# shyam196/egc

Hardware: AMD Instinct MI355X
Metric: EGC-M layer fwd edges/sec on ogbn-arxiv; achieved HBM GB/s vs roofline (higher is better)
Workload: dtype f32

## Files before the change

egc_amd/csrc/egc_aggregate.hip:

```cpp
#include <stdlib.h>

#include <algorithm>

#include "egc_aggregate_dev.h"
#include "egc_pack_map.h"

namespace egc {

bool stdvar_reference(const egc_layer* layer) {
  const char* e = getenv("EGC_STDVAR_REFERENCE");
  if (layer == nullptr || e == nullptr || e[0] == '\0' || (e[0] == '0' && e[1] == '\0')) return false;
  for (int t = 0; t < layer->num_aggrs && t < EGC_MAX_AGGRS; ++t)
    if (layer->aggrs[t] == EGC_AGGR_VAR || layer->aggrs[t] == EGC_AGGR_STD) return true;
  return false;
}

template <int CHUNKS>
__device__ inline void set_shift(const AggArgs& a, __amdgpu_buffer_rsrc_t rsrc, int row, int lane, Acc<CHUNKS>& acc) {
  bool need = false;
  for (int t = 0; t < a.A; ++t) need = need || a.aggr[t] == EGC_AGGR_VAR || a.aggr[t] == EGC_AGGR_STD;
  if (!need && a.stats == nullptr) return;
  if (a.var_ref) return;
  const int rs = __builtin_amdgcn_readfirstlane(a.rowptr[row]), re = __builtin_amdgcn_readfirstlane(a.rowptr[row + 1]);
  if (re <= rs) return;
  const int first = __builtin_amdgcn_readfirstlane(a.col[rs]);
  const int q = lane & ((1 << a.lpr_log2) - 1);
#pragma unroll
  for (int k = 0; k < CHUNKS; ++k) {
    const int s = k * 64 + q;
    acc.sh[k] = load_slot(rsrc, s < a.slots ? (unsigned)first * (unsigned)a.ldb * 4u + (unsigned)s * 16u : OOB);
  }
}

template <int CHUNKS, int U>
__device__ inline void accumulate_range(const AggArgs& a, __amdgpu_buffer_rsrc_t rsrc, int row, int start, int end,
                                        int lane, Acc<CHUNKS>& acc, int& nself) {
  const int G = 64 >> a.lpr_log2;
// ... 661 lines not shown
  PlanCaps caps = plan_caps(n, e);
  a.rows_per_wave = 0;
  a.n_chunks_hint = (graph->n_chunks >= 0 && graph->n_chunks <= caps.cap_chunks) ? (int)graph->n_chunks : -1;
  const bool force_generic = getenv("EGC_FORCE_GENERIC") != nullptr || a.var_ref != 0;
  if (!force_generic && fast_path_supported(a, layer->weight_layout, chunks)) {
    if (arg_done != nullptr) *arg_done = true;
    return launch_fast(a, n, caps, stream);
  }

  switch (chunks) {
    case 1: return launch_all<1>(a, n, caps, wpb, lds_bytes, stream);
    case 2: return launch_all<2>(a, n, caps, wpb, lds_bytes, stream,
                                 !force_generic && getenv("EGC_NO_WIDE") == nullptr && wide_path_supported(a, layer->weight_layout));
    case 3: return launch_all<3>(a, n, caps, wpb, lds_bytes, stream);
    case 4: return launch_all<4>(a, n, caps, wpb, lds_bytes, stream);
    default: return EGC_ERR_UNSUPPORTED;
  }
}

int egc_layer_forward_f32(const egc_graph* graph, const egc_layer* layer, const float* x, const float* wcat,
                          const float* bcat, const float* bias, float* bases, int32_t ldb, float* weightings,
                          float* out, void* workspace, size_t workspace_bytes, egc_stream_t stream) {
  if (graph == nullptr) return EGC_ERR_INVALID;
  int st = validate_layer(layer);
  if (st != EGC_OK) return st;
  const int fg = layer->num_bases * layer_basis_stride(layer);
  const int w = layer->num_heads * layer->num_bases * layer->num_aggrs;
  st = egc_basis_transform_f32(x, wcat, bcat, graph->n_nodes, layer->in_channels, fg, w, bases, ldb, weightings, stream);
  if (st != EGC_OK) return st;
  return egc_aggregate_combine_f32(graph, layer, bases, ldb, weightings, bias, out, nullptr, nullptr, workspace,
                                   workspace_bytes, stream);
}

int egc_layer_forward_packed(const egc_graph* graph, const egc_layer* layer, const float* x, const void* packed,
                             const float* bcat, const float* bias, float* bases, int32_t ldb, float* weightings,
                             float* out, void* workspace, size_t workspace_bytes, egc_stream_t stream) {
  if (graph == nullptr) return EGC_ERR_INVALID;
  int st = validate_layer(layer);
  if (st != EGC_OK) return st;
  const int fg = layer->num_bases * layer_basis_stride(layer);
  const int w = layer->num_heads * layer->num_bases * layer->num_aggrs;
  st = egc_basis_transform_packed_ex(x, packed, bcat, graph->n_nodes, layer->in_channels, fg, w, egc_layer_gemm_flags(layer),
                                     bases, ldb, weightings, stream);
  if (st != EGC_OK) return st;
  return egc_aggregate_combine_f32(graph, layer, bases, ldb, weightings, bias, out, nullptr, nullptr, workspace,
                                   workspace_bytes, stream);
}

static int tile_layer_args(const egc_layer* layer, AggArgs& a, bool two_sets_ok = false) {
  int st = validate_layer(layer);
  if (st != EGC_OK) return st;
  a = AggArgs{};
  a.ldb = egc_bases_ld(layer);
  a.slots = a.ldb / 4;
  a.F_out = layer->out_channels;
  a.H = layer->num_heads;
  a.B = layer->num_bases;
  a.A = layer->num_aggrs;
  a.L = layer->out_channels / layer->num_heads;
  a.Ls = layer_basis_stride(layer);
  a.W = a.H * a.B * a.A;
  a.ldw = a.W;
  for (int t = 0; t < EGC_MAX_AGGRS; ++t) a.aggr[t] = t < a.A ? layer->aggrs[t] : 0;
  a.x_looped = layer->agg_set == EGC_SET_LOOPED;
  a.y_looped = layer->sym_set == EGC_SET_LOOPED;
  a.loops_all = layer->loops_all_nodes != 0;
  if (layer->weight_layout == EGC_LAYOUT_HAB) { a.sa = a.B; a.sb = 1; } else { a.sa = 1; a.sb = a.A; }
  a.act = layer->weight_act;
  a.lpr_log2 = 4;
  int chunks = a.slots <= 64 ? 1 : (a.slots + 63) / 64;
  a.n_nodes = 1;
  if (!fast_path_supported(a, layer->weight_layout, chunks) && !(two_sets_ok && wide_path_supported(a, layer->weight_layout)))
    return EGC_ERR_UNSUPPORTED;
  return EGC_OK;
// ... 230 lines not shown
```

egc_amd/csrc/egc_aggregate_fast.hip:

```cpp
#include <stdlib.h>

#include "egc_aggregate_fast_dev.h"

namespace egc {

template <int LPR_LOG2, int HPB, int NEED, class C>
#ifndef EGC_AGG_WAVES_SQ
#define EGC_AGG_WAVES_SQ 5
#endif
__global__ void __launch_bounds__(256) __attribute__((amdgpu_waves_per_eu(NEED == 0 ? EGC_AGG_WAVES : ((NEED & NEED_ARG) && (NEED & NEED_SQ)) ? 2 : (NEED == NEED_SQ || NEED == NEED_MN) ? EGC_AGG_WAVES_SQ : 4)))
agg_fast_kernel(AggArgs a) {
  constexpr int LPR = 1 << LPR_LOG2, G = 64 / LPR;
  extern __shared__ float smem[];
  if ((int)blockIdx.x < a.chunk_blocks && (int)blockIdx.x * 4 >= a.plan[1]) return;
  const int wave = __builtin_amdgcn_readfirstlane(threadIdx.x >> 6);
  const int lane = threadIdx.x & 63;
  const int g = lane >> LPR_LOG2;
  const int q = lane & (LPR - 1);
  const unsigned slot_off = (unsigned)q * 16u;
  const unsigned row_bytes = (unsigned)a.ldb * 4u;
  const bool lane_live = q < C::slots(a);
  const int F_out = C::F_out(a);
  float* lds_bias = smem + wave * a.lds_floats_per_wave;
  const bool post = a.post_scale != nullptr;
// ... 483 lines not shown
  const int lpr = a.slots <= 16 ? 16 : a.slots <= 32 ? 32 : 64;
  const int G = 64 / lpr;
  a.lanes_pb = a.Ls / 4;
  a.magic_P = (unsigned)(((uint64_t)1 << 32) / (uint64_t)a.lanes_pb) + 1u;
  if ((a.lanes_pb & (a.lanes_pb - 1)) == 0) {
    int lg = 0;
    while ((4 << lg) < a.Ls) ++lg;
    a.lpb_log2 = lg;
  } else {
    a.lpb_log2 = -1;
  }
  if (a.rows_per_wave <= 0) a.rows_per_wave = (G == 1 && (int64_t)a.row_end - a.row_begin >= 32768) ? 4 : 1;
  if (a.rows_per_wave * G > 60) a.rows_per_wave = 60 / G;
  a.chunk_blocks = (int)ceil_div(a.n_chunks_hint >= 0 ? a.n_chunks_hint : caps.cap_chunks, 4);
  a.need_mean = a.need_var = 0;
  int need = 0;
  for (int t = 0; t < a.A; ++t) {
    if (a.aggr[t] == EGC_AGGR_MEAN || a.aggr[t] == EGC_AGGR_VAR || a.aggr[t] == EGC_AGGR_STD) a.need_mean = 1;
    if (a.aggr[t] == EGC_AGGR_VAR || a.aggr[t] == EGC_AGGR_STD) { a.need_var = 1; need |= NEED_SQ; }
    if (a.aggr[t] == EGC_AGGR_MIN) need |= NEED_MN;
  }
  a.w_lds_stride = (a.W + 3) & ~3;
  a.bias_lds_floats = (a.H * a.Ls + 3) & ~3;
  a.lds_floats_per_wave = (a.post_scale != nullptr ? 2 : 1) * a.bias_lds_floats + G * a.w_lds_stride;
  size_t lds = (size_t)4 * a.lds_floats_per_wave * sizeof(float);
  if (lds > 64 * 1024) return EGC_ERR_UNSUPPORTED;
  const int64_t row_blocks = ceil_div((int64_t)a.row_end - a.row_begin, (int64_t)4 * a.rows_per_wave * G);
  const unsigned grid = (unsigned)(a.chunk_blocks + row_blocks);

  if (getenv("EGC_NO_STATIC_CFG") == nullptr) {
    int status = EGC_OK;
    constexpr int S = EGC_AGGR_SUM, M = EGC_AGGR_MEAN, X = EGC_AGGR_MAX, Y = EGC_AGGR_SYMNORM;
    EGC_STATIC_CFG(8, 4, 16, 4, agg_pack(S, M, X, Y), EGC_ACT_NONE, true, true, true, 0)
    EGC_STATIC_CFG(8, 4, 16, 4, agg_pack(S, EGC_AGGR_STD, X, Y), EGC_ACT_NONE, true, true, true, NEED_SQ)
    EGC_STATIC_CFG(8, 4, 16, 1, agg_pack(Y), EGC_ACT_NONE, true, true, true, 0)
    EGC_STATIC_CFG(8, 4, 16, 3, agg_pack(Y, X, M), EGC_ACT_NONE, false, true, true, 0)
    EGC_STATIC_CFG(8, 4, 16, 1, agg_pack(Y), EGC_ACT_NONE, false, true, true, 0)
    EGC_STATIC_CFG(8, 4, 23, 1, agg_pack(Y), EGC_ACT_NONE, false, true, true, 0)
    EGC_STATIC_CFG(4, 4, 34, 3, agg_pack(Y, X, M), EGC_ACT_NONE, false, true, true, 0)
    EGC_STATIC_CFG(8, 4, 21, 1, agg_pack(Y), EGC_ACT_NONE, false, true, true, 0)
    EGC_STATIC_CFG(4, 4, 31, 3, agg_pack(S, EGC_AGGR_STD, X), EGC_ACT_NONE, false, true, true, NEED_SQ)
    EGC_STATIC_CFG(4, 4, 32, 3, agg_pack(Y, EGC_AGGR_STD, X), EGC_ACT_NONE, false, true, true, NEED_SQ)
    EGC_STATIC_CFG(8, 4, 37, 1, agg_pack(Y), EGC_ACT_NONE, false, true, true, 0)
    EGC_STATIC_CFG(4, 4, 56, 3, agg_pack(S, M, X), EGC_ACT_NONE, false, true, true, 0)
    EGC_STATIC_CFG(8, 4, 44, 1, agg_pack(Y), EGC_ACT_NONE, true, true, true, 0)
    EGC_STATIC_CFG(8, 4, 44, 1, agg_pack(M), EGC_ACT_NONE, true, true, true, 0)
    EGC_STATIC_CFG(8, 4, 16, 2, agg_pack(M, X), EGC_ACT_NONE, false, false, true, 0)
    EGC_STATIC_CFG(8, 4, 16, 1, agg_pack(S), EGC_ACT_NONE, false, false, true, 0)
    EGC_STATIC_CFG(4, 4, 16, 2, agg_pack(M, X), EGC_ACT_NONE, false, false, true, 0)
    EGC_STATIC_CFG(4, 4, 16, 1, agg_pack(S), EGC_ACT_NONE, false, false, true, 0)
  }
  switch (lpr) {
    case 16: return launch_rt<4>(a, need, grid, lds, stream);
    case 32: return launch_rt<5>(a, need, grid, lds, stream);
    default: return launch_rt<6>(a, need, grid, lds, stream);
  }
}

}
```

egc_amd/csrc/egc_gemm_bf16x3.hip:

```cpp
#include <stdlib.h>

#include <algorithm>

#include "egc_common.h"
#include <stdio.h>

#include "egc_gemm_split.h"

namespace egc {

typedef float f32x16 __attribute__((ext_vector_type(16)));
typedef __bf16 bf16x8 __attribute__((ext_vector_type(8)));
typedef unsigned short u16;
typedef unsigned int u32x4 __attribute__((ext_vector_type(4)));
typedef unsigned int u32x2 __attribute__((ext_vector_type(2)));
typedef float f32x4v __attribute__((ext_vector_type(4)));

constexpr int XBM = 128;
constexpr int XBN = 192;
constexpr int XKT = 32;
constexpr int XLD = 40;

__device__ inline void lds_barrier() {
  asm volatile("s_waitcnt lgkmcnt(0)\n\ts_barrier" ::: "memory");
// ... 447 lines not shown
  int buf = 0;
  for (; tile < n_tiles; tile += stride) {
    load_tile(tile + stride, xr);
    compute_tile(tile, buf);
    if (tile + stride < n_tiles) stage_tile(buf ^ 1, xr);
    lds_barrier();
    buf ^= 1;
  }
}

template <int KSUB>
static int launch_ws(const float* x, const u16* packed, const float* bcat, int64_t M, int K, int W, float* bases, int ldb,
                     float* weightings, int NV, hipStream_t stream) {
  const int nt = NV / 32;
  const int threads = 64 * nt;
  const int pieces = WS_ROWS * (16 * KSUB) / 4;
  if (threads * 4 < pieces) return EGC_ERR_UNSUPPORTED;
  const int64_t n_tiles64 = ceil_div(M, WS_ROWS);
  if (n_tiles64 >= ((int64_t)1 << 31)) return EGC_ERR_INVALID;
  const int n_tiles = (int)n_tiles64;
  const size_t lds = (size_t)2 * 3 * WS_ROWS * (16 * KSUB + 8) * sizeof(u16);
  int blocks_per_cu = nt <= 4 ? 4 : (nt <= 8 ? 2 : 1);
  int grid = 256 * blocks_per_cu;
  if (grid > n_tiles) grid = n_tiles;
  const int x_vec4 = (K % 4 == 0) && ((reinterpret_cast<uintptr_t>(x) & 15) == 0);
  basis_gemm_ws_kernel<KSUB><<<grid, threads, lds, stream>>>(x, packed, bcat, M, K, W, bases, ldb, weightings, NV, n_tiles,
                                                             x_vec4);
  EGC_LAUNCH_CHECK("basis_gemm_ws_kernel");
  return EGC_OK;
}

static inline int round_up32(int v) { return (v + 31) & ~31; }

}

using namespace egc;

extern "C" {

size_t egc_basis_pack_bytes(int32_t f_in, int32_t f_g, int32_t w_cols) {
  if (f_in <= 0 || f_g <= 0 || w_cols < 0) return 0;
  const int ldb = (f_g + 3) & ~3;
  const int NV = round_up32(ldb + w_cols);
  const int KS = (f_in + XKT - 1) / XKT;
  return std::max(std::max((size_t)KS * 3 * NV * XKT * sizeof(u16), f16x2_pack_bytes(KS, NV)),
                  f16x2k_pack_bytes(f_in, f_g, ldb, w_cols));
}

static bool use_f16x2(int f_in, int ldb, int NV, int flags, int w_cols) {
  return (flags & EGC_GEMM_24BIT) == 0 && f16x2_shape(f_in, ldb, NV, w_cols);
}
static bool use_f16x2k(int f_in, int f_g, int ldb, int w_cols, int flags) {
  return (flags & EGC_GEMM_24BIT) == 0 && f16x2k_shape(f_in, f_g, ldb, w_cols);
}

static int basis_pack_strided(const float* wcat, int64_t rs, int64_t cs, int32_t f_in, int32_t f_g, int32_t w_cols,
                              void* packed, size_t packed_bytes, hipStream_t stream, int flags = 0) {
  if (wcat == nullptr || packed == nullptr || f_in <= 0 || f_g <= 0 || w_cols < 0) return EGC_ERR_INVALID;
  if (packed_bytes < egc_basis_pack_bytes(f_in, f_g, w_cols)) return EGC_ERR_WORKSPACE;
  const int ldb = (f_g + 3) & ~3;
  const int NV = round_up32(ldb + w_cols);
  const int KS = (f_in + XKT - 1) / XKT;
  if (use_f16x2(f_in, ldb, NV, flags, w_cols)) return f16x2_pack(wcat, rs, cs, f_in, f_g, w_cols, ldb, NV, KS, packed, stream);
  if (use_f16x2k(f_in, f_g, ldb, w_cols, flags)) return f16x2k_pack(wcat, rs, cs, f_in, f_g, ldb, w_cols, packed, stream);
  const int total = KS * NV * XKT;
  pack_bf16x3_kernel<<<(total + 255) / 256, 256, 0, stream>>>(wcat, rs, cs, f_in, f_g, w_cols, ldb, NV, KS, (u16*)packed);
// ... 107 lines not shown
```

egc_amd/csrc/egc_gemm_f16x2.hip:

```cpp
#include <stdlib.h>

#include <algorithm>
#include <cstdio>
#include <vector>

#include "egc_common.h"
#include "egc_gemm_split.h"

namespace egc {

typedef float f32x16 __attribute__((ext_vector_type(16)));
typedef _Float16 f16x8 __attribute__((ext_vector_type(8)));
typedef _Float16 f16x2 __attribute__((ext_vector_type(2)));
typedef float f32x2 __attribute__((ext_vector_type(2)));
typedef float f32x4v __attribute__((ext_vector_type(4)));
typedef unsigned short u16;
typedef unsigned int u32x4 __attribute__((ext_vector_type(4)));
typedef unsigned int u32x2 __attribute__((ext_vector_type(2)));

__device__ inline void lds_barrier2() { asm volatile("s_waitcnt lgkmcnt(0)\n\ts_barrier" ::: "memory"); }

constexpr int F16X2_KP = 128;

__device__ inline void scales_of(unsigned amax_bits, float& scale, float& inv) {
// ... 13 lines not shown
__global__ void __launch_bounds__(64) pack_f16x2_kernel(const float* __restrict__ wcat, int64_t rs, int64_t cs, int K, int F_g,
                                                        int W, int ldb, int NV, int KS, u16* __restrict__ packed) {
  const int v = blockIdx.x;
  const int lane = threadIdx.x;
  const int src = (v < F_g) ? v : ((v < ldb || v >= ldb + W) ? -1 : v - ldb + F_g);
  unsigned amax = 0;
  if (src >= 0)
    for (int k = lane; k < K; k += 64) amax = max(amax, __float_as_uint(wcat[k * rs + src * cs]) & 0x7fffffffu);
#pragma unroll
  for (int d = 32; d >= 1; d >>= 1) amax = max(amax, (unsigned)__shfl_xor((int)amax, d));
  float scale, inv;
  scales_of(amax, scale, inv);
  for (int k = lane; k < KS * GEMM_KT; k += 64) {
    const float w = (src >= 0 && k < K) ? wcat[k * rs + src * cs] * scale : 0.f;
    const _Float16 h = (_Float16)w;
    const _Float16 l = (_Float16)((w - (float)h) * 2048.f);
    const int64_t base = ((((int64_t)(v >> 5) * (F16X2_KP / 16) + (k >> 4)) * 2) * 64 + 32 * ((k & 15) >> 3) + (v & 31)) * 8 + (k & 7);
    packed[base] = __builtin_bit_cast(u16, h);
    packed[base + 64 * 8] = __builtin_bit_cast(u16, l);
  }
  if (lane == 0) reinterpret_cast<float*>(packed + (int64_t)KS * 2 * NV * GEMM_KT)[v] = inv;
}

#ifdef EGC_GEMM_STAMPS
__device__ unsigned long long* egc_stamp_buf2 = nullptr;
#endif

constexpr int F16X2_THREADS = 768;
constexpr int F16X2_ROWS = 64;
constexpr int F16X2_LDX = F16X2_KP + 8;
constexpr int F16X2_RAW_BYTES = F16X2_ROWS * F16X2_KP * 4;
constexpr int F16X2_PLANE_BYTES = 2 * 2 * F16X2_ROWS * F16X2_LDX * 2;
constexpr int F16X2_STORES_PER_TILE = 16;

#define EGC_VMCNT(n) asm volatile("s_waitcnt vmcnt(%0)" ::"n"(n) : "memory")

__global__ void __launch_bounds__(F16X2_THREADS) basis_gemm_f16x2_kernel(const float* __restrict__ x,
                                                                          const u16* __restrict__ packed,
                                                                          const float* __restrict__ bcat, int64_t M, int K,
                                                                          int W, float* __restrict__ bases, int ldb,
                                                                          float* __restrict__ weightings, int NV,
                                                                          int rows_per_block) {
  constexpr int KP = F16X2_KP;
  constexpr int KSUB = KP / 16;
  constexpr int LDX = F16X2_LDX;
  constexpr int ROWS = F16X2_ROWS;
  constexpr int XBUF = 2 * ROWS * LDX;
  constexpr int nthreads = F16X2_THREADS;
  extern __shared__ __attribute__((aligned(16))) u16 smem_h2[];
  u16* xs = smem_h2;
  char* raw = reinterpret_cast<char*>(smem_h2) + F16X2_PLANE_BYTES;
  float* row_inv = reinterpret_cast<float*>(raw + 2 * F16X2_RAW_BYTES);
  const int tid = threadIdx.x;
  const int lane = tid & 63;
  const int wave = __builtin_amdgcn_readfirstlane(tid >> 6);
  const int ct = wave % 6, rt = wave / 6;
#ifdef EGC_GEMM_STAMPS
  unsigned long long t_entry;
  asm volatile("s_memrealtime %0\n\ts_waitcnt lgkmcnt(0)" : "=s"(t_entry) :: "memory");
#endif
  const int l31 = lane & 31, hh = lane >> 5;
  const int cb = 32 * ct;
  const int64_t row_lo = (int64_t)blockIdx.x * rows_per_block;
  const int64_t row_hi = row_lo + rows_per_block < M ? row_lo + rows_per_block : M;
  const int n_tiles = (int)((row_hi - row_lo + F16X2_ROWS - 1) / F16X2_ROWS);

  f16x8 wf[KSUB][2];
  float col_inv, col_bias;
  constexpr unsigned GOOB = 0xFFFFFFF0u;
  constexpr unsigned SOOB = 0x80000000u;
  const u32x4 rx = {(unsigned)(uintptr_t)x, (unsigned)((uintptr_t)x >> 32) & 0xffffu, (unsigned)(M * K * 4), 0x00020000u};
  const bool to_bases = cb < ldb;
  const __amdgpu_buffer_rsrc_t ro =
      to_bases ? __builtin_amdgcn_make_buffer_rsrc((void*)bases, 0, (unsigned)(row_hi * ldb * 4), 0x00020000)
               : __builtin_amdgcn_make_buffer_rsrc((void*)weightings, 0, (unsigned)(row_hi * (int64_t)W * 4), 0x00020000);
  const int out_ld = to_bases ? ldb : W;
  const int out_col = (to_bases ? cb : cb - ldb) + l31;
#if defined(EGC_DIAG_GEMM_NO_W_STORE) || defined(EGC_DIAG_GEMM_NO_W)
  const bool col_ok = to_bases && out_col < ldb;
#else
  const bool col_ok = out_col < (to_bases ? ldb : W);
#endif
  const unsigned raw_lds = (unsigned)(uintptr_t)raw;
  const bool third = wave < 8;

  auto dma_piece = [&](int tile, int slot, int i) {
    const int pc = tid + nthreads * i;
    const int row = pc >> 5;
    const int k4 = (pc & 31) * 4;
    const int64_t gm = row_lo + (int64_t)tile * ROWS + row;
    const bool ok = (tile < n_tiles) & (gm < row_hi) & (k4 < K);
    const unsigned voff = ok ? (unsigned)((gm * K + k4) * 4) : GOOB;
    const unsigned dst =
        __builtin_amdgcn_readfirstlane(raw_lds + slot * F16X2_RAW_BYTES + (wave * 64 + nthreads * i) * 16);
    unsigned keep;
    asm volatile("s_mov_b32 %0, m0\n\ts_mov_b32 m0, %2\n\ts_nop 0\n\tbuffer_load_dwordx4 %1, %3, 0 offen lds\n\ts_mov_b32 m0, %0"
                 : "=&s"(keep)
                 : "v"(voff), "s"(dst), "s"(rx)
                 : "memory");
  };
  auto dma_tile = [&](int tile, int slot) {
    dma_piece(tile, slot, 0);
    dma_piece(tile, slot, 1);
    if (third) dma_piece(tile, slot, 2);
  };
  auto row_amax = [&](const float4 v) -> unsigned {
    float m;
    asm("v_max3_f32 %0, |%1|, |%2|, |%3|\n\tv_max_f32 %0, |%4|, %0" : "=&v"(m) : "v"(v.x), "v"(v.y), "v"(v.z), "v"(v.w));
    unsigned a = __float_as_uint(m);
    a = max(a, (unsigned)__builtin_amdgcn_update_dpp(0, (int)a, 0xB1, 0xf, 0xf, true));
    a = max(a, (unsigned)__builtin_amdgcn_update_dpp(0, (int)a, 0x4E, 0xf, 0xf, true));
    a = max(a, (unsigned)__builtin_amdgcn_update_dpp(0, (int)a, 0x141, 0xf, 0xf, true));
    a = max(a, (unsigned)__builtin_amdgcn_update_dpp(0, (int)a, 0x140, 0xf, 0xf, true));
    return max(a, (unsigned)__builtin_amdgcn_ds_swizzle((int)a, 0x401F));
  };
  auto split_store = [&](int buf, int ri, int i, const float4 v, unsigned amax) {
    const int pc = tid + nthreads * i;
    const int row = pc >> 5;
    const int k4 = (pc & 31) * 4;
    unsigned e = amax & 0x7f800000u;
    e = min(max(e, 13u << 23), 253u << 23);
    const float sc = __uint_as_float(0x7f000000u - e);
    const float sc2k = __uint_as_float(0x7f000000u + (11u << 23) - e);
    const f16x2 h01 = __builtin_convertvector(f32x2{v.x * sc, v.y * sc}, f16x2);
    const f16x2 h23 = __builtin_convertvector(f32x2{v.z * sc, v.w * sc}, f16x2);
    f16x2 l01, l23;
    l01[0] = (_Float16)__builtin_fmaf((float)h01[0], -2048.f, v.x * sc2k);
    l01[1] = (_Float16)__builtin_fmaf((float)h01[1], -2048.f, v.y * sc2k);
    l23[0] = (_Float16)__builtin_fmaf((float)h23[0], -2048.f, v.z * sc2k);
    l23[1] = (_Float16)__builtin_fmaf((float)h23[1], -2048.f, v.w * sc2k);
    u16* dst = xs + buf * XBUF + row * LDX + k4;
    *reinterpret_cast<u32x2*>(dst) = u32x2{__builtin_bit_cast(unsigned, h01), __builtin_bit_cast(unsigned, h23)};
    *reinterpret_cast<u32x2*>(dst + ROWS * LDX) = u32x2{__builtin_bit_cast(unsigned, l01), __builtin_bit_cast(unsigned, l23)};
    row_inv[ri * ROWS + row] = __uint_as_float(e);
  };
  auto raw_piece = [&](int slot, int i) -> float4 {
    return *reinterpret_cast<const float4*>(raw + slot * F16X2_RAW_BYTES + (tid + nthreads * i) * 16);
  };
  auto stage = [&](int buf, int ri, int slot, int i) {
    const float4 v = raw_piece(slot, i);
    split_store(buf, ri, i, v, row_amax(v));
  };
  auto frag = [&](int buf, int s, f16x8& xh, f16x8& xl) {
    const u16* xb = xs + buf * XBUF + (32 * rt + l31) * LDX + 16 * s + 8 * hh;
    xh = *reinterpret_cast<const f16x8*>(xb);
    xl = *reinterpret_cast<const f16x8*>(xb + ROWS * LDX);
  };
  f32x16 acc0, acc1, t;
  auto mfma_step = [&](int s, const f16x8 xh, const f16x8 xl) {
#ifdef EGC_DIAG_GEMM_NO_W
    if (!to_bases) return;
#endif
    acc0 = __builtin_amdgcn_mfma_f32_32x32x16_f16(xh, wf[s][0], acc0, 0, 0, 0);
    acc1 = __builtin_amdgcn_mfma_f32_32x32x16_f16(xl, wf[s][0], acc1, 0, 0, 0);
    acc1 = __builtin_amdgcn_mfma_f32_32x32x16_f16(xh, wf[s][1], acc1, 0, 0, 0);
  };
  auto epilogue = [&](unsigned voff, int j, const float* rinv_t) {
    const float4 ri = *reinterpret_cast<const float4*>(rinv_t + 32 * rt + 8 * j + 4 * hh);
    const float v0 = __builtin_fmaf(t[4 * j], col_inv * ri.x, col_bias);
    const float v1 = __builtin_fmaf(t[4 * j + 1], col_inv * ri.y, col_bias);
    const float v2 = __builtin_fmaf(t[4 * j + 2], col_inv * ri.z, col_bias);
    const float v3 = __builtin_fmaf(t[4 * j + 3], col_inv * ri.w, col_bias);
    const int so = (8 * j) * out_ld * 4;
    __builtin_amdgcn_raw_buffer_store_b32(__float_as_uint(v0), ro, voff, so, 0);
    __builtin_amdgcn_raw_buffer_store_b32(__float_as_uint(v1), ro, voff, so + out_ld * 4, 0);
    __builtin_amdgcn_raw_buffer_store_b32(__float_as_uint(v2), ro, voff, so + 2 * out_ld * 4, 0);
    __builtin_amdgcn_raw_buffer_store_b32(__float_as_uint(v3), ro, voff, so + 3 * out_ld * 4, 0);
  };
  auto out_offset = [&](int tile, bool valid) -> unsigned {
    return (valid & col_ok) ? (unsigned)(((row_lo + (int64_t)tile * ROWS + 32 * rt + 4 * hh) * out_ld + out_col) * 4) : SOOB;
  };
#define EGC_PIN __builtin_amdgcn_sched_barrier(0)

  constexpr int stride = 1;
  int tile = 0;
  if (n_tiles <= 0) return;
  if (K < KP) {
    for (int i = tid; i < 2 * F16X2_RAW_BYTES / 16; i += nthreads) reinterpret_cast<u32x4*>(raw)[i] = u32x4{0, 0, 0, 0};
    lds_barrier2();
  }
  dma_tile(tile, 0);
  dma_tile(tile + stride, 1);
#ifdef EGC_GEMM_STAMPS
  unsigned long long t_a, t_b;
  asm volatile("s_memrealtime %0\n\ts_waitcnt lgkmcnt(0)" : "=s"(t_a) :: "memory");
#endif
#pragma unroll
  for (int s = 0; s < KSUB; ++s)
#pragma unroll
    for (int p = 0; p < 2; ++p) {
      wf[s][p] = *reinterpret_cast<const f16x8*>(packed + ((((int64_t)ct * KSUB + s) * 2 + p) * 64 + lane) * 8);
    }
  col_inv = reinterpret_cast<const float*>(packed + (int64_t)(KP / GEMM_KT) * 2 * NV * GEMM_KT)[cb + l31];
  const int wcol = cb + l31 - ldb;
  col_bias = (bcat != nullptr && wcol >= 0 && wcol < W) ? bcat[wcol] : 0.f;
  EGC_VMCNT(0);
  asm volatile("" : "+v"(wf[0][0]), "+v"(wf[0][1]), "+v"(wf[1][0]), "+v"(wf[1][1]), "+v"(wf[2][0]), "+v"(wf[2][1]),
               "+v"(wf[3][0]), "+v"(wf[3][1]), "+v"(wf[4][0]), "+v"(wf[4][1]), "+v"(wf[5][0]), "+v"(wf[5][1]),
               "+v"(wf[6][0]), "+v"(wf[6][1]), "+v"(wf[7][0]), "+v"(wf[7][1]), "+v"(col_inv), "+v"(col_bias));
#ifdef EGC_GEMM_STAMPS
  asm volatile("s_memrealtime %0\n\ts_waitcnt lgkmcnt(0)" : "=s"(t_b) :: "memory");
#endif
  stage(0, 0, 0, 0);
  stage(0, 0, 0, 1);
  if (third) stage(0, 0, 0, 2);
  dma_tile(tile + 2 * stride, 0);
  lds_barrier2();
  int buf = 0;
  int ri_cur = 0;
  unsigned prev_off = SOOB;
  const float* prev_ri = row_inv;
#pragma unroll
  for (int r = 0; r < 16; ++r) t[r] = 0.f;
#ifdef EGC_GEMM_STAMPS
  unsigned long long tsum[6] = {0, 0, 0, 0, 0, 0}, t0, t1, r0, r1;
#define EGC_STAMP(k) { asm volatile("s_memtime %0\n\ts_waitcnt lgkmcnt(0)" : "=s"(t1) :: "memory"); tsum[k] += t1 - t0; t0 = t1; }
  asm volatile("s_memrealtime %0\n\ts_waitcnt lgkmcnt(0)" : "=s"(r0) :: "memory");
  asm volatile("s_memtime %0\n\ts_waitcnt lgkmcnt(0)" : "=s"(t0) :: "memory");
#else
#define EGC_STAMP(k)
#endif
  static_assert(F16X2_STORES_PER_TILE == 16, "vmcnt count below");
  for (; tile < n_tiles; tile += stride) {
    const int slot = buf ^ 1;
    const int ri_next = ri_cur == 2 ? 0 : ri_cur + 1;
    f16x8 xh, xl, yh, yl;
    frag(buf, 0, xh, xl);
#pragma unroll
    for (int r = 0; r < 16; ++r) { acc0[r] = 0.f; acc1[r] = 0.f; }
    frag(buf, 1, yh, yl);
    mfma_step(0, xh, xl);
    epilogue(prev_off, 0, prev_ri);
    EGC_PIN;
    frag(buf, 2, xh, xl);
    mfma_step(1, yh, yl);
    epilogue(prev_off, 1, prev_ri);
    EGC_PIN;
    frag(buf, 3, yh, yl);
    mfma_step(2, xh, xl);
    epilogue(prev_off, 2, prev_ri);
    EGC_PIN;
    frag(buf, 4, xh, xl);
    mfma_step(3, yh, yl);
    epilogue(prev_off, 3, prev_ri);
    EGC_PIN;
    EGC_STAMP(0)
    EGC_VMCNT(34);
    frag(buf, 5, yh, yl);
    mfma_step(4, xh, xl);
    stage(buf ^ 1, ri_next, slot, 0);
    EGC_PIN;
    frag(buf, 6, xh, xl);
    mfma_step(5, yh, yl);
    stage(buf ^ 1, ri_next, slot, 1);
    EGC_PIN;
    frag(buf, 7, yh, yl);
    mfma_step(6, xh, xl);
    if (third) stage(buf ^ 1, ri_next, slot, 2);
    EGC_PIN;
    mfma_step(7, yh, yl);
    dma_tile(tile + 3 * stride, slot);
    EGC_PIN;
    EGC_STAMP(1)
#pragma unroll
    for (int r = 0; r < 16; ++r) t[r] = __builtin_fmaf(acc1[r], 1.f / 2048.f, acc0[r]);
    prev_off = out_offset(tile, true);
    prev_ri = row_inv + ri_cur * ROWS;
    ri_cur = ri_cur == 2 ? 0 : ri_cur + 1;
    EGC_STAMP(2)
    lds_barrier2();
    EGC_STAMP(3)
    buf ^= 1;
  }
  epilogue(prev_off, 0, prev_ri);
  epilogue(prev_off, 1, prev_ri);
  epilogue(prev_off, 2, prev_ri);
  epilogue(prev_off, 3, prev_ri);
  EGC_VMCNT(0);
#ifdef EGC_GEMM_STAMPS
  asm volatile("s_memrealtime %0\n\ts_waitcnt lgkmcnt(0)" : "=s"(r1) :: "memory");
  tsum[5] = r1 - r0;
  if (lane == 0 && egc_stamp_buf2 != nullptr) {
    for (int k = 0; k < 6; ++k) egc_stamp_buf2[(blockIdx.x * 16 + wave) * 6 + k] = tsum[k];
    egc_stamp_buf2[1024 * 16 * 6 + (blockIdx.x * 16 + wave) * 2] = t_entry;
    egc_stamp_buf2[1024 * 16 * 6 + (blockIdx.x * 16 + wave) * 2 + 1] = r1;
    egc_stamp_buf2[(blockIdx.x * 16 + wave) * 6 + 4] = r0 - t_entry;
    egc_stamp_buf2[(blockIdx.x * 16 + wave) * 6 + 3] = ((t_a - t_entry) << 32) | (t_b - t_entry);
  }
#endif
}

size_t f16x2_pack_bytes(int KS, int NV) { return (size_t)KS * 2 * NV * GEMM_KT * sizeof(u16) + (size_t)NV * sizeof(float); }

int f16x2_pack(const float* wcat, int64_t rs, int64_t cs, int f_in, int f_g, int w_cols, int ldb, int NV, int KS, void* packed,
               hipStream_t stream) {
  pack_f16x2_kernel<<<NV, 64, 0, stream>>>(wcat, rs, cs, f_in, f_g, w_cols, ldb, NV, KS, (u16*)packed);
  EGC_LAUNCH_CHECK("pack_f16x2_kernel");
  return EGC_OK;
}

static int f16x2_launch_rows(const float* x, const void* packed, const float* bcat, int64_t M, int K, int W, float* bases,
                             int ldb, float* weightings, int NV, hipStream_t stream) {
  constexpr int ROWS = F16X2_ROWS;
  const int threads = F16X2_THREADS;
  const int64_t n_tiles64 = (M + ROWS - 1) / ROWS;
  if (n_tiles64 >= ((int64_t)1 << 31)) return EGC_ERR_INVALID;
  const int n_tiles = (int)n_tiles64;
  const size_t lds = (size_t)F16X2_PLANE_BYTES + 2 * (size_t)F16X2_RAW_BYTES + (size_t)(3 * ROWS) * sizeof(float);
  static bool attr_set = false;
  if (!attr_set) {
    hipError_t e = hipFuncSetAttribute(reinterpret_cast<const void*>(&basis_gemm_f16x2_kernel),
                                       hipFuncAttributeMaxDynamicSharedMemorySize, 160 * 1024);
    if (e != hipSuccess) { set_last_error("hipFuncSetAttribute(f16x2)", e); return EGC_ERR_HIP; }
    attr_set = true;
  }
  int grid = 256;
  if (grid > n_tiles) grid = n_tiles;
  const int rows_per_block = (int)((M + grid - 1) / grid);
#ifdef EGC_GEMM_STAMPS
  static unsigned long long* dbuf = nullptr;
  if (dbuf == nullptr) {
    hipMalloc(&dbuf, 1024 * 16 * 8 * 8);
    hipMemcpyToSymbol(HIP_SYMBOL(egc_stamp_buf2), &dbuf, sizeof(dbuf));
  }
  hipMemset(dbuf, 0, 1024 * 16 * 8 * 8);
#endif
  basis_gemm_f16x2_kernel<<<grid, threads, lds, stream>>>(x, (const u16*)packed, bcat, M, K, W, bases, ldb, weightings,
                                                               NV, rows_per_block);
  EGC_LAUNCH_CHECK("basis_gemm_f16x2_kernel");
#ifdef EGC_GEMM_STAMPS
  {
    hipDeviceSynchronize();
    static int calls = 0;
    if (++calls == 20) {
      std::vector<unsigned long long> h(1024 * 16 * 8);
      hipMemcpy(h.data(), dbuf, h.size() * 8, hipMemcpyDeviceToHost);
      double sum[6] = {0, 0, 0, 0, 0, 0}; int nw = 0;
      for (int b = 0; b < grid; ++b)
        for (int w = 0; w < threads / 64; ++w) {
          for (int k = 0; k < 6; ++k) sum[k] += (double)h[(b * 16 + w) * 6 + k];
          ++nw;
        }
      {
        unsigned long long lo = ~0ull, hi = 0; int early = 0;
        for (int b = 0; b < grid; ++b) { unsigned long long e = h[1024 * 16 * 6 + (b * 16) * 2]; if (e && e < lo) lo = e; }
        for (int b = 0; b < grid; ++b) {
          unsigned long long e = h[1024 * 16 * 6 + (b * 16) * 2], x = h[1024 * 16 * 6 + (b * 16) * 2 + 1];
          if (x > hi) hi = x;
          if (e - lo < 300) ++early;
        }
        double pro = 0, lmin = 1e30, lmax = 0, pa = 0, pb = 0;
        for (int b = 0; b < grid; ++b) {
          pro += (double)h[(b * 16) * 6 + 4];
          pa += (double)(h[(b * 16) * 6 + 3] >> 32); pb += (double)(h[(b * 16) * 6 + 3] & 0xffffffffull);
          lmin = std::min(lmin, (double)h[(b * 16) * 6 + 5]);
          lmax = std::max(lmax, (double)h[(b * 16) * 6 + 5]);
        }
        fprintf(stderr, "[stamps f16x2] kernel span %.1f us, %d of %d blocks entered within 3 us; prologue avg %.1f us (dma issued %.1f, all landed %.1f); loop min %.1f max %.1f us\n",
                (hi - lo) * 0.01, early, grid, pro / grid * 0.01, pa / grid * 0.01, pb / grid * 0.01, lmin * 0.01, lmax * 0.01);
      }
      const double tpb = (double)n_tiles / grid;
      const double cyc = sum[0] + sum[1] + sum[2] + sum[3];
      fprintf(stderr, "[stamps f16x2] per tile per wave (cycles): k0-3+epi %.0f  k4-7+stage %.0f  t-fma %.0f  barrier %.0f  (-) %.0f "
              "(tiles/block %.1f)  clock %.2f GHz  loop %.1f us\n", sum[0] / nw / tpb, sum[1] / nw / tpb, sum[2] / nw / tpb,
              sum[3] / nw / tpb, sum[4] / nw / tpb, tpb, cyc / sum[5] * 0.1, sum[5] / nw * 0.01);
    }
  }
#endif
  return EGC_OK;
}

int f16x2_launch(const float* x, const void* packed, const float* bcat, int64_t M, int K, int W, float* bases, int ldb,
                 float* weightings, int NV, hipStream_t stream) {
  if (NV != 192 || K > F16X2_KP || K % 4 != 0 || (ldb % 32 != 0 && W != 0) || (reinterpret_cast<uintptr_t>(x) & 15) != 0)
    return EGC_ERR_UNSUPPORTED;
  const int64_t widest = std::max(std::max(K, ldb), W);
  int64_t max_rows = ((int64_t)0x7FFFFFF0 / (4 * widest)) & ~(int64_t)(F16X2_ROWS - 1);
  if (const char* e = getenv("EGC_GEMM_MAX_ROWS")) max_rows = std::max<int64_t>(F16X2_ROWS, atoll(e) & ~(int64_t)(F16X2_ROWS - 1));
  for (int64_t r0 = 0; r0 < M; r0 += max_rows) {
    const int64_t rows = std::min(max_rows, M - r0);
    const int st = f16x2_launch_rows(x + r0 * K, packed, bcat, rows, K, W, bases + r0 * ldb, ldb,
                                     weightings != nullptr ? weightings + r0 * W : nullptr, NV, stream);
    if (st != EGC_OK) return st;
  }
  return EGC_OK;
}

}
```

egc_amd/csrc/egc_gemm_split.h:

```cpp
#pragma once
#include <hip/hip_runtime.h>
#include <stddef.h>
#include <stdint.h>

namespace egc {

constexpr int GEMM_KT = 32;

inline bool f16x2_shape(int f_in, int ldb, int NV, int w_cols) {
  return f_in > 96 && f_in <= 128 && f_in % 4 == 0 && NV == 192 && (ldb % 32 == 0 || w_cols == 0);
}

size_t f16x2_pack_bytes(int KS, int NV);
int f16x2_pack(const float* wcat, int64_t rs, int64_t cs, int f_in, int f_g, int w_cols, int ldb, int NV, int KS, void* packed,
               hipStream_t stream);
int f16x2_launch(const float* x, const void* packed, const float* bcat, int64_t M, int K, int W, float* bases, int ldb,
                 float* weightings, int NV, hipStream_t stream);

bool f16x2k_shape(int f_in, int f_g, int ldb, int w_cols);
size_t f16x2k_pack_bytes(int f_in, int f_g, int ldb, int w_cols);
int f16x2k_pack(const float* wcat, int64_t rs, int64_t cs, int f_in, int f_g, int ldb, int w_cols, void* packed,
                hipStream_t stream);
int f16x2k_launch(const float* x, const void* packed, const float* bcat, int64_t M, int K, int f_g, int ldb, int W,
                  float* bases, float* weightings, hipStream_t stream, const float* addend = nullptr);

}
```

Before: 17.93 billion.

## Fold mean aggregator into sum weighting inside basis GEMM epilogue

When a layer has sum, mean and symnorm aggregators, mean equals sum scaled by inverse degree, so the GEMM epilogue adds the mean weighting times 1/deg (recovered from dis) into the sum weighting column and drops the mean column. The aggregation kernel then runs with three aggregators, cutting weighting writes and reads and per-edge accumulation work. The cost is extra DMA of dis per tile, DPP lane shuffles in the epilogue, a templated kernel, and reliance on degree being recoverable from rint(1/dis^2).

```diff
diff --git a/egc_amd/csrc/egc_aggregate.hip b/egc_amd/csrc/egc_aggregate.hip
--- a/egc_amd/csrc/egc_aggregate.hip
+++ b/egc_amd/csrc/egc_aggregate.hip
@@ -3,6 +3,7 @@
 #include <algorithm>
 
 #include "egc_aggregate_dev.h"
+#include "egc_gemm_split.h"
 #include "egc_pack_map.h"
 
 namespace egc {
@@ -730,6 +731,23 @@
                                    workspace_bytes, stream);
 }
 
+static bool fold_mean(const egc_graph* graph, const egc_layer* layer, int* fs, int* fm, const float** dis) {
+  if (layer->num_aggrs != 4 || layer->weight_layout != EGC_LAYOUT_HBA || layer->weight_act != EGC_ACT_NONE) return false;
+  int s = -1, m = -1, y = 0;
+  for (int t = 0; t < 4; ++t) {
+    const int c = layer->aggrs[t];
+    if (c == EGC_AGGR_SUM) s = s < 0 ? t : 4;
+    if (c == EGC_AGGR_MEAN) m = m < 0 ? t : 4;
+    if (c == EGC_AGGR_SYMNORM) y = 1;
+  }
+  if (s < 0 || m < 0 || s > 3 || m > 3 || !y || layer->sym_set != layer->agg_set) return false;
+  *dis = layer->agg_set == EGC_SET_LOOPED ? graph->dis_looped : graph->dis_raw;
+  if (*dis == nullptr) return false;
+  *fs = s;
+  *fm = m;
+  return true;
+}
+
 int egc_layer_forward_packed(const egc_graph* graph, const egc_layer* layer, const float* x, const void* packed,
                              const float* bcat, const float* bias, float* bases, int32_t ldb, float* weightings,
                              float* out, void* workspace, size_t workspace_bytes, egc_stream_t stream) {
@@ -738,6 +756,21 @@
   if (st != EGC_OK) return st;
   const int fg = layer->num_bases * layer_basis_stride(layer);
   const int w = layer->num_heads * layer->num_bases * layer->num_aggrs;
+  int fs, fm;
+  const float* dis;
+  if (fold_mean(graph, layer, &fs, &fm, &dis)) {
+    st = egc::basis_transform_packed_folded(x, packed, bcat, graph->n_nodes, layer->in_channels, fg, w, egc_layer_gemm_flags(layer),
+                                            bases, ldb, weightings, dis, fs, fm, (hipStream_t)stream);
+    if (st == EGC_OK) {
+      egc_layer folded = *layer;
+      folded.num_aggrs = 3;
+      for (int t = fm; t < 3; ++t) folded.aggrs[t] = layer->aggrs[t + 1];
+      folded.aggrs[3] = 0;
+      return egc_aggregate_combine_f32(graph, &folded, bases, ldb, weightings, bias, out, nullptr, nullptr, workspace,
+                                       workspace_bytes, stream);
+    }
+    if (st != EGC_ERR_UNSUPPORTED) return st;
+  }
   st = egc_basis_transform_packed_ex(x, packed, bcat, graph->n_nodes, layer->in_channels, fg, w, egc_layer_gemm_flags(layer),
                                      bases, ldb, weightings, stream);
   if (st != EGC_OK) return st;
diff --git a/egc_amd/csrc/egc_aggregate_fast.hip b/egc_amd/csrc/egc_aggregate_fast.hip
--- a/egc_amd/csrc/egc_aggregate_fast.hip
+++ b/egc_amd/csrc/egc_aggregate_fast.hip
@@ -539,6 +539,7 @@
     int status = EGC_OK;
     constexpr int S = EGC_AGGR_SUM, M = EGC_AGGR_MEAN, X = EGC_AGGR_MAX, Y = EGC_AGGR_SYMNORM;
     EGC_STATIC_CFG(8, 4, 16, 4, agg_pack(S, M, X, Y), EGC_ACT_NONE, true, true, true, 0)
+    EGC_STATIC_CFG(8, 4, 16, 3, agg_pack(S, X, Y), EGC_ACT_NONE, true, true, true, 0)
     EGC_STATIC_CFG(8, 4, 16, 4, agg_pack(S, EGC_AGGR_STD, X, Y), EGC_ACT_NONE, true, true, true, NEED_SQ)
     EGC_STATIC_CFG(8, 4, 16, 1, agg_pack(Y), EGC_ACT_NONE, true, true, true, 0)
     EGC_STATIC_CFG(8, 4, 16, 3, agg_pack(Y, X, M), EGC_ACT_NONE, false, true, true, 0)
diff --git a/egc_amd/csrc/egc_gemm_bf16x3.hip b/egc_amd/csrc/egc_gemm_bf16x3.hip
--- a/egc_amd/csrc/egc_gemm_bf16x3.hip
+++ b/egc_amd/csrc/egc_gemm_bf16x3.hip
@@ -503,6 +503,17 @@
 
 static inline int round_up32(int v) { return (v + 31) & ~31; }
 
+int basis_transform_packed_folded(const float* x, const void* packed, const float* bcat, int64_t n_nodes, int32_t f_in,
+                                  int32_t f_g, int32_t w_cols, int32_t flags, float* bases, int32_t ldb, float* weightings,
+                                  const float* dis, int fold_s, int fold_m, hipStream_t stream) {
+  if (n_nodes < 0 || f_in <= 0 || f_g <= 0 || w_cols <= 0 || ldb != ((f_g + 3) & ~3)) return EGC_ERR_INVALID;
+  if (x == nullptr || packed == nullptr || bases == nullptr || weightings == nullptr || dis == nullptr) return EGC_ERR_INVALID;
+  const int NV = round_up32(ldb + w_cols);
+  if ((flags & EGC_GEMM_24BIT) != 0 || !f16x2_shape(f_in, ldb, NV, w_cols) || w_cols % 32 != 0) return EGC_ERR_UNSUPPORTED;
+  if (n_nodes == 0) return EGC_OK;
+  return f16x2_launch(x, packed, bcat, n_nodes, f_in, w_cols, bases, ldb, weightings, NV, stream, dis, fold_s, fold_m);
+}
+
 }
 
 using namespace egc;
diff --git a/egc_amd/csrc/egc_gemm_f16x2.hip b/egc_amd/csrc/egc_gemm_f16x2.hip
--- a/egc_amd/csrc/egc_gemm_f16x2.hip
+++ b/egc_amd/csrc/egc_gemm_f16x2.hip
@@ -69,15 +69,20 @@
 constexpr int F16X2_RAW_BYTES = F16X2_ROWS * F16X2_KP * 4;
 constexpr int F16X2_PLANE_BYTES = 2 * 2 * F16X2_ROWS * F16X2_LDX * 2;
 constexpr int F16X2_STORES_PER_TILE = 16;
+constexpr int F16X2_CNT_SLOTS = 8;
+constexpr int F16X2_LDS_BYTES = F16X2_PLANE_BYTES + 2 * F16X2_RAW_BYTES + 3 * F16X2_ROWS * 4 + (F16X2_CNT_SLOTS * F16X2_ROWS + 4) * 4;
+
 
 #define EGC_VMCNT(n) asm volatile("s_waitcnt vmcnt(%0)" ::"n"(n) : "memory")
 
+template <int FM>
 __global__ void __launch_bounds__(F16X2_THREADS) basis_gemm_f16x2_kernel(const float* __restrict__ x,
                                                                           const u16* __restrict__ packed,
                                                                           const float* __restrict__ bcat, int64_t M, int K,
                                                                           int W, float* __restrict__ bases, int ldb,
                                                                           float* __restrict__ weightings, int NV,
-                                                                          int rows_per_block) {
+                                                                          int rows_per_block, const float* __restrict__ dis,
+                                                                          int fold_s) {
   constexpr int KP = F16X2_KP;
   constexpr int KSUB = KP / 16;
   constexpr int LDX = F16X2_LDX;
@@ -88,6 +93,8 @@
   u16* xs = smem_h2;
   char* raw = reinterpret_cast<char*>(smem_h2) + F16X2_PLANE_BYTES;
   float* row_inv = reinterpret_cast<float*>(raw + 2 * F16X2_RAW_BYTES);
+  float* icnt = row_inv + 3 * ROWS;
+  float* zero4 = icnt + F16X2_CNT_SLOTS * ROWS;
   const int tid = threadIdx.x;
   const int lane = tid & 63;
   const int wave = __builtin_amdgcn_readfirstlane(tid >> 6);
@@ -108,16 +115,27 @@
   constexpr unsigned SOOB = 0x80000000u;
   const u32x4 rx = {(unsigned)(uintptr_t)x, (unsigned)((uintptr_t)x >> 32) & 0xffffu, (unsigned)(M * K * 4), 0x00020000u};
   const bool to_bases = cb < ldb;
+  const int wcol_v = cb - ldb + l31;
+  const int qa = wcol_v & 3;
+#ifdef EGC_DIAG_FOLD_W128
+  constexpr int FMS = -1;
+#else
+  constexpr int FMS = FM;
+#endif
+  const int W_out = FMS >= 0 ? W / 4 * 3 : W;
   const __amdgpu_buffer_rsrc_t ro =
       to_bases ? __builtin_amdgcn_make_buffer_rsrc((void*)bases, 0, (unsigned)(row_hi * ldb * 4), 0x00020000)
-               : __builtin_amdgcn_make_buffer_rsrc((void*)weightings, 0, (unsigned)(row_hi * (int64_t)W * 4), 0x00020000);
-  const int out_ld = to_bases ? ldb : W;
-  const int out_col = (to_bases ? cb : cb - ldb) + l31;
+               : __builtin_amdgcn_make_buffer_rsrc((void*)weightings, 0, (unsigned)(row_hi * (int64_t)W_out * 4), 0x00020000);
+  const int out_ld = to_bases ? ldb : W_out;
+  const int out_col = to_bases ? cb + l31 : FMS >= 0 ? 3 * (wcol_v >> 2) + qa - (qa > FMS ? 1 : 0) : wcol_v;
 #if defined(EGC_DIAG_GEMM_NO_W_STORE) || defined(EGC_DIAG_GEMM_NO_W)
   const bool col_ok = to_bases && out_col < ldb;
 #else
-  const bool col_ok = out_col < (to_bases ? ldb : W);
-#endif
+  const bool col_ok = to_bases ? out_col < ldb : (wcol_v < W && (FMS < 0 || qa != FMS));
+#endif
+  const bool is_sum = FM >= 0 && !to_bases && qa == fold_s;
+  const u32x4 rd = {(unsigned)(uintptr_t)dis, (unsigned)((uintptr_t)dis >> 32) & 0xffffu, (unsigned)(M * 4), 0x00020000u};
+  const unsigned icnt_lds = (unsigned)(uintptr_t)icnt;
   const unsigned raw_lds = (unsigned)(uintptr_t)raw;
   const bool third = wave < 8;
 
@@ -136,10 +154,28 @@
                  : "v"(voff), "s"(dst), "s"(rx)
                  : "memory");
   };
+  auto dma_cnt = [&](int tile) {
+    const int64_t gm = row_lo + (int64_t)tile * ROWS + lane;
+    const bool ok = (tile < n_tiles) & (gm < row_hi);
+    const unsigned voff = ok ? (unsigned)(gm * 4) : GOOB;
+    const unsigned dst = __builtin_amdgcn_readfirstlane(icnt_lds + (tile & (F16X2_CNT_SLOTS - 1)) * ROWS * 4);
+    unsigned keep;
+    asm volatile("s_mov_b32 %0, m0\n\ts_mov_b32 m0, %2\n\ts_nop 0\n\tbuffer_load_dword %1, %3, 0 offen lds\n\ts_mov_b32 m0, %0"
+                 : "=&s"(keep)
+                 : "v"(voff), "s"(dst), "s"(rd)
+                 : "memory");
+  };
   auto dma_tile = [&](int tile, int slot) {
     dma_piece(tile, slot, 0);
     dma_piece(tile, slot, 1);
     if (third) dma_piece(tile, slot, 2);
+    if (FM >= 0 && wave == 8) dma_cnt(tile);
+  };
+  auto cnt_inverse = [&](int tile) {
+    float* p = icnt + (tile & (F16X2_CNT_SLOTS - 1)) * ROWS + lane;
+    const float d = *p;
+    const float c = __builtin_rintf(__builtin_amdgcn_rcpf(d * d));
+    *p = __builtin_amdgcn_rcpf(fmaxf(c, 1.f));
   };
   auto row_amax = [&](const float4 v) -> unsigned {
     float m;
@@ -192,12 +228,26 @@
     acc1 = __builtin_amdgcn_mfma_f32_32x32x16_f16(xl, wf[s][0], acc1, 0, 0, 0);
     acc1 = __builtin_amdgcn_mfma_f32_32x32x16_f16(xh, wf[s][1], acc1, 0, 0, 0);
   };
-  auto epilogue = [&](unsigned voff, int j, const float* rinv_t) {
+  auto epilogue = [&](unsigned voff, int j, const float* rinv_t, const float* icnt_t) {
     const float4 ri = *reinterpret_cast<const float4*>(rinv_t + 32 * rt + 8 * j + 4 * hh);
-    const float v0 = __builtin_fmaf(t[4 * j], col_inv * ri.x, col_bias);
-    const float v1 = __builtin_fmaf(t[4 * j + 1], col_inv * ri.y, col_bias);
-    const float v2 = __builtin_fmaf(t[4 * j + 2], col_inv * ri.z, col_bias);
-    const float v3 = __builtin_fmaf(t[4 * j + 3], col_inv * ri.w, col_bias);
+    float v0 = __builtin_fmaf(t[4 * j], col_inv * ri.x, col_bias);
+    float v1 = __builtin_fmaf(t[4 * j + 1], col_inv * ri.y, col_bias);
+    float v2 = __builtin_fmaf(t[4 * j + 2], col_inv * ri.z, col_bias);
+    float v3 = __builtin_fmaf(t[4 * j + 3], col_inv * ri.w, col_bias);
+#ifdef EGC_DIAG_FOLD_NO_MATH
+    if constexpr (false) {
+#else
+    if constexpr (FM >= 0) {
+#endif
+      if (!to_bases) {
+        const float4 ic = *reinterpret_cast<const float4*>(is_sum ? icnt_t + 32 * rt + 8 * j + 4 * hh : zero4);
+        constexpr int QP = FM | (FM << 2) | (FM << 4) | (FM << 6);
+        v0 = __builtin_fmaf(__int_as_float(__builtin_amdgcn_update_dpp(0, __float_as_int(v0), QP, 0xf, 0xf, false)), ic.x, v0);
+        v1 = __builtin_fmaf(__int_as_float(__builtin_amdgcn_update_dpp(0, __float_as_int(v1), QP, 0xf, 0xf, false)), ic.y, v1);
+        v2 = __builtin_fmaf(__int_as_float(__builtin_amdgcn_update_dpp(0, __float_as_int(v2), QP, 0xf, 0xf, false)), ic.z, v2);
+        v3 = __builtin_fmaf(__int_as_float(__builtin_amdgcn_update_dpp(0, __float_as_int(v3), QP, 0xf, 0xf, false)), ic.w, v3);
+      }
+    }
     const int so = (8 * j) * out_ld * 4;
     __builtin_amdgcn_raw_buffer_store_b32(__float_as_uint(v0), ro, voff, so, 0);
     __builtin_amdgcn_raw_buffer_store_b32(__float_as_uint(v1), ro, voff, so + out_ld * 4, 0);
@@ -212,6 +262,7 @@
   constexpr int stride = 1;
   int tile = 0;
   if (n_tiles <= 0) return;
+  if (FM >= 0 && tid < 4) zero4[tid] = 0.f;
   if (K < KP) {
     for (int i = tid; i < 2 * F16X2_RAW_BYTES / 16; i += nthreads) reinterpret_cast<u32x4*>(raw)[i] = u32x4{0, 0, 0, 0};
     lds_barrier2();
@@ -247,6 +298,7 @@
   int ri_cur = 0;
   unsigned prev_off = SOOB;
   const float* prev_ri = row_inv;
+  const float* prev_ic = icnt;
 #pragma unroll
   for (int r = 0; r < 16; ++r) t[r] = 0.f;
 #ifdef EGC_GEMM_STAMPS
@@ -267,22 +319,23 @@
     for (int r = 0; r < 16; ++r) { acc0[r] = 0.f; acc1[r] = 0.f; }
     frag(buf, 1, yh, yl);
     mfma_step(0, xh, xl);
-    epilogue(prev_off, 0, prev_ri);
+    epilogue(prev_off, 0, prev_ri, prev_ic);
     EGC_PIN;
     frag(buf, 2, xh, xl);
     mfma_step(1, yh, yl);
-    epilogue(prev_off, 1, prev_ri);
+    epilogue(prev_off, 1, prev_ri, prev_ic);
     EGC_PIN;
     frag(buf, 3, yh, yl);
     mfma_step(2, xh, xl);
-    epilogue(prev_off, 2, prev_ri);
+    epilogue(prev_off, 2, prev_ri, prev_ic);
     EGC_PIN;
     frag(buf, 4, xh, xl);
     mfma_step(3, yh, yl);
-    epilogue(prev_off, 3, prev_ri);
+    epilogue(prev_off, 3, prev_ri, prev_ic);
     EGC_PIN;
     EGC_STAMP(0)
     EGC_VMCNT(34);
+    if (FM >= 0 && wave == 8) cnt_inverse(tile);
     frag(buf, 5, yh, yl);
     mfma_step(4, xh, xl);
     stage(buf ^ 1, ri_next, slot, 0);
@@ -303,16 +356,17 @@
     for (int r = 0; r < 16; ++r) t[r] = __builtin_fmaf(acc1[r], 1.f / 2048.f, acc0[r]);
     prev_off = out_offset(tile, true);
     prev_ri = row_inv + ri_cur * ROWS;
+    prev_ic = icnt + (tile & (F16X2_CNT_SLOTS - 1)) * ROWS;
     ri_cur = ri_cur == 2 ? 0 : ri_cur + 1;
     EGC_STAMP(2)
     lds_barrier2();
     EGC_STAMP(3)
     buf ^= 1;
   }
-  epilogue(prev_off, 0, prev_ri);
-  epilogue(prev_off, 1, prev_ri);
-  epilogue(prev_off, 2, prev_ri);
-  epilogue(prev_off, 3, prev_ri);
+  epilogue(prev_off, 0, prev_ri, prev_ic);
+  epilogue(prev_off, 1, prev_ri, prev_ic);
+  epilogue(prev_off, 2, prev_ri, prev_ic);
+  epilogue(prev_off, 3, prev_ri, prev_ic);
   EGC_VMCNT(0);
 #ifdef EGC_GEMM_STAMPS
   asm volatile("s_memrealtime %0\n\ts_waitcnt lgkmcnt(0)" : "=s"(r1) :: "memory");
@@ -336,21 +390,33 @@
   return EGC_OK;
 }
 
+template <int FM>
+static int f16x2_launch_fm(int grid, size_t lds, const float* x, const void* packed, const float* bcat, int64_t M, int K, int W,
+                           float* bases, int ldb, float* weightings, int NV, int rows_per_block, const float* dis, int fold_s,
+                           hipStream_t stream) {
+  static bool attr_set = false;
+  if (!attr_set) {
+    hipError_t e = hipFuncSetAttribute(reinterpret_cast<const void*>(&basis_gemm_f16x2_kernel<FM>),
+                                       hipFuncAttributeMaxDynamicSharedMemorySize, 160 * 1024);
+    if (e != hipSuccess) { set_last_error("hipFuncSetAttribute(f16x2)", e); return EGC_ERR_HIP; }
+    attr_set = true;
+  }
+  basis_gemm_f16x2_kernel<FM><<<grid, F16X2_THREADS, lds, stream>>>(x, (const u16*)packed, bcat, M, K, W, bases, ldb, weightings,
+                                                                    NV, rows_per_block, dis, fold_s);
+  EGC_LAUNCH_CHECK("basis_gemm_f16x2_kernel");
+  return EGC_OK;
+}
+
 static int f16x2_launch_rows(const float* x, const void* packed, const float* bcat, int64_t M, int K, int W, float* bases,
-                             int ldb, float* weightings, int NV, hipStream_t stream) {
+                             int ldb, float* weightings, int NV, const float* dis, int fold_s, int fold_m, hipStream_t stream) {
   constexpr int ROWS = F16X2_ROWS;
   const int threads = F16X2_THREADS;
+  (void)threads;
   const int64_t n_tiles64 = (M + ROWS - 1) / ROWS;
   if (n_tiles64 >= ((int64_t)1 << 31)) return EGC_ERR_INVALID;
   const int n_tiles = (int)n_tiles64;
-  const size_t lds = (size_t)F16X2_PLANE_BYTES + 2 * (size_t)F16X2_RAW_BYTES + (size_t)(3 * ROWS) * sizeof(float);
-  static bool attr_set = false;
-  if (!attr_set) {
-    hipError_t e = hipFuncSetAttribute(reinterpret_cast<const void*>(&basis_gemm_f16x2_kernel),
-                                       hipFuncAttributeMaxDynamicSharedMemorySize, 160 * 1024);
-    if (e != hipSuccess) { set_last_error("hipFuncSetAttribute(f16x2)", e); return EGC_ERR_HIP; }
-    attr_set = true;
-  }
+  const size_t lds = (size_t)F16X2_LDS_BYTES;
+  static_assert(F16X2_LDS_BYTES <= 160 * 1024, "LDS of one CU");
   int grid = 256;
   if (grid > n_tiles) grid = n_tiles;
   const int rows_per_block = (int)((M + grid - 1) / grid);
@@ -362,9 +428,15 @@
   }
   hipMemset(dbuf, 0, 1024 * 16 * 8 * 8);
 #endif
-  basis_gemm_f16x2_kernel<<<grid, threads, lds, stream>>>(x, (const u16*)packed, bcat, M, K, W, bases, ldb, weightings,
-                                                               NV, rows_per_block);
-  EGC_LAUNCH_CHECK("basis_gemm_f16x2_kernel");
+  int st;
+  switch (fold_m) {
+    case 0: st = f16x2_launch_fm<0>(grid, lds, x, packed, bcat, M, K, W, bases, ldb, weightings, NV, rows_per_block, dis, fold_s, stream); break;
+    case 1: st = f16x2_launch_fm<1>(grid, lds, x, packed, bcat, M, K, W, bases, ldb, weightings, NV, rows_per_block, dis, fold_s, stream); break;
+    case 2: st = f16x2_launch_fm<2>(grid, lds, x, packed, bcat, M, K, W, bases, ldb, weightings, NV, rows_per_block, dis, fold_s, stream); break;
+    case 3: st = f16x2_launch_fm<3>(grid, lds, x, packed, bcat, M, K, W, bases, ldb, weightings, NV, rows_per_block, dis, fold_s, stream); break;
+    default: st = f16x2_launch_fm<-1>(grid, lds, x, packed, bcat, M, K, W, bases, ldb, weightings, NV, rows_per_block, nullptr, -1, stream);
+  }
+  if (st != EGC_OK) return st;
 #ifdef EGC_GEMM_STAMPS
   {
     hipDeviceSynchronize();
@@ -408,16 +480,20 @@
 }
 
 int f16x2_launch(const float* x, const void* packed, const float* bcat, int64_t M, int K, int W, float* bases, int ldb,
-                 float* weightings, int NV, hipStream_t stream) {
+                 float* weightings, int NV, hipStream_t stream, const float* dis, int fold_s, int fold_m) {
   if (NV != 192 || K > F16X2_KP || K % 4 != 0 || (ldb % 32 != 0 && W != 0) || (reinterpret_cast<uintptr_t>(x) & 15) != 0)
     return EGC_ERR_UNSUPPORTED;
+  const bool fold = fold_m >= 0;
+  if (fold && (dis == nullptr || W % 32 != 0 || fold_m > 3 || fold_s < 0 || fold_s > 3 || fold_s == fold_m)) return EGC_ERR_INVALID;
+  const int W_out = fold ? W / 4 * 3 : W;
   const int64_t widest = std::max(std::max(K, ldb), W);
   int64_t max_rows = ((int64_t)0x7FFFFFF0 / (4 * widest)) & ~(int64_t)(F16X2_ROWS - 1);
   if (const char* e = getenv("EGC_GEMM_MAX_ROWS")) max_rows = std::max<int64_t>(F16X2_ROWS, atoll(e) & ~(int64_t)(F16X2_ROWS - 1));
   for (int64_t r0 = 0; r0 < M; r0 += max_rows) {
     const int64_t rows = std::min(max_rows, M - r0);
     const int st = f16x2_launch_rows(x + r0 * K, packed, bcat, rows, K, W, bases + r0 * ldb, ldb,
-                                     weightings != nullptr ? weightings + r0 * W : nullptr, NV, stream);
+                                     weightings != nullptr ? weightings + r0 * W_out : nullptr, NV, fold ? dis + r0 : nullptr,
+                                     fold_s, fold ? fold_m : -1, stream);
     if (st != EGC_OK) return st;
   }
   return EGC_OK;
diff --git a/egc_amd/csrc/egc_gemm_split.h b/egc_amd/csrc/egc_gemm_split.h
--- a/egc_amd/csrc/egc_gemm_split.h
+++ b/egc_amd/csrc/egc_gemm_split.h
@@ -15,7 +15,10 @@
 int f16x2_pack(const float* wcat, int64_t rs, int64_t cs, int f_in, int f_g, int w_cols, int ldb, int NV, int KS, void* packed,
                hipStream_t stream);
 int f16x2_launch(const float* x, const void* packed, const float* bcat, int64_t M, int K, int W, float* bases, int ldb,
-                 float* weightings, int NV, hipStream_t stream);
+                 float* weightings, int NV, hipStream_t stream, const float* dis = nullptr, int fold_s = -1, int fold_m = -1);
+int basis_transform_packed_folded(const float* x, const void* packed, const float* bcat, int64_t n_nodes, int32_t f_in,
+                                  int32_t f_g, int32_t w_cols, int32_t flags, float* bases, int32_t ldb, float* weightings,
+                                  const float* dis, int fold_s, int fold_m, hipStream_t stream);
 
 bool f16x2k_shape(int f_in, int f_g, int ldb, int w_cols);
 size_t f16x2k_pack_bytes(int f_in, int f_g, int ldb, int w_cols);
```

Result: faster. 18.49 billion, median of 6 (+3.1%).
